# alexanderswerdlow/BEVGen

Measured on AMD Instinct MI355X. Metric: multi-view scenes/sec (6x256x256), higher is better.
Workload: dtype f32 (GEMM/conv/attention products as 3 f16 MFMAs on hi/lo splits, fp32 accumulate); 1 GPU; BASELINE configs[1]: Route M MaskGit, 6x256x256, batch 16 scenes/GPU, 18 iterations, + VQGAN decode to uint8; global_batch=16, parallelism=scene-parallel x1 (RCCL gather of uint8 pixels), precision_mode=f16x3

## Files before the change

### bevgen_amd/csrc/gemm_split_glds.hip

```cpp
#include "common.h"
#include "kernels.h"
#include "profiler.h"
#include <type_traits>
#include <vector>
#include <cstdio>

namespace bevgen {

typedef _Float16 half8 __attribute__((ext_vector_type(8)));
typedef unsigned u32x4 __attribute__((ext_vector_type(4)));

struct RowDiv {
    float d, r;
    __device__ __forceinline__ explicit RowDiv(float d_) : d(d_) {
        float r0 = __builtin_amdgcn_rcpf(d_);
        const float e = fmaf(-d_, r0, 1.0f);
        r0 = fmaf(e, r0, r0);
        const float e2 = fmaf(-d_, r0, 1.0f);
        r = fmaf(e2, r0, r0);
    }
    __device__ __forceinline__ float operator()(float x) const {
        const float q0 = x * r;
        const float e = fmaf(-d, q0, x);
        return fmaf(e, r, q0);
    }
};
constexpr int GBN = 128, GBK = 32;
#ifdef BEVGEN_GEMM_TRACE
__device__ unsigned long long g_gemm_trace[5 * 2048 * 8];
__device__ unsigned long long g_gemm_tr_tmp[2];
#define GT_STAMP(i) do { if (MODE == MODE_PLAIN && !KS) gt[i] = __builtin_amdgcn_s_memrealtime(); } while (0)
#else
#define GT_STAMP(i) do { } while (0)
#endif
constexpr float kGLoInv = 1.f / 2048.f;

__device__ __forceinline__ void glds16(const _Float16* src, _Float16* lds_wave_base) {
    __builtin_amdgcn_global_load_lds((const __attribute__((address_space(1))) void*)src, (__attribute__((address_space(3))) void*)lds_wave_base, 16, 0, 0);
}
__device__ __forceinline__ void glds16_buf(__amdgpu_buffer_rsrc_t rsrc, unsigned voff, int soff, _Float16* lds_wave_base) {
    __builtin_amdgcn_raw_ptr_buffer_load_lds(rsrc, (__attribute__((address_space(3))) void*)lds_wave_base, 16, (int)voff, soff, 0, 0);
}
template <int N>
__device__ __forceinline__ void wait_vmcnt() { asm volatile("s_waitcnt vmcnt(%0)" ::"n"(N) : "memory"); }
template <int DMA, int MAXN>
__device__ __forceinline__ void wait_tiles(int n) {
    if constexpr (MAXN <= 0) wait_vmcnt<0>();
    else {
        if (n >= MAXN) wait_vmcnt<MAXN * DMA>();
        else wait_tiles<DMA, MAXN - 1>(n);
    }
}

template <int DMA, int MAXN, int X>
__device__ __forceinline__ void wait_tiles_x(int n) {
    if constexpr (MAXN <= 0) wait_vmcnt<X>();
    else {
        if (n >= MAXN) wait_vmcnt<MAXN * DMA + X>();
        else wait_tiles_x<DMA, MAXN - 1, X>(n);
    }
}

template <int MODE, int WM, int S, bool W16, bool KS, int TI, int TJ, bool SKK = false>
__device__ __forceinline__ void gemm_tile(const GemmArgs& g, const int tx, const int ty, const int kt_first, const int nk, const int ksl, const int kz, const int sk_role,
                                          const int sk_first, const int tid
#ifdef BEVGEN_GEMM_TRACE
                                          , unsigned long long* gt
#endif
                                          ) {
    constexpr int TBM = WM * 64;
    constexpr int NW = WM * 8 / (TI * TJ);
    constexpr int WROWS = TI * 32;
    constexpr int WCOLS = TJ * 32;
    constexpr int WN = GBN / WCOLS;
    constexpr int NAJ = TBM / 8 / NW;
    constexpr int NBJ = 16 / NW;
    constexpr int AREGION = TBM * 2 * GBK;
    constexpr int STAGE_H = AREGION + GBN * 2 * GBK;
    constexpr int DMA = NAJ + NBJ;
    extern __shared__ __attribute__((aligned(1024))) _Float16 smem_g[];
    const int lane = tid & 63;
    const int wave = __builtin_amdgcn_readfirstlane(tid >> 6);
    const int wm = wave / WN, wn = wave % WN;
    const int r = lane & 31, h = lane >> 5;
    const int n0 = tx * GBN, m0 = ty * TBM + g.m_base;
    const int n0l = n0, m0l = m0;

    const _Float16* Ap = reinterpret_cast<const _Float16*>(g.A_hi);
    const _Float16* Bp = reinterpret_cast<const _Float16*>(g.B_hi);

    constexpr bool CONVG = MODE == MODE_CONV3, CONVS = MODE == MODE_CONV3S, CONV = CONVG || CONVS;
    unsigned a_off[NAJ], b_off[NBJ];
    int a_img[CONVG ? NAJ : 1], a_yx[CONVG ? NAJ : 1];
    unsigned a_msk[CONVS ? NAJ : 1];
#pragma unroll
    for (int j = 0; j < NBJ; ++j) {
        const int R = wave * (8 * NBJ) + j * 8 + (lane >> 3);
        const int c = (lane & 7) ^ ((R >> 1) & 7);
        const int n = min(n0l + R, g.N - 1);
        b_off[j] = (unsigned)(((long)n * 2 * g.ldb + c * 8) * 2);
    }
#pragma unroll
    for (int j = 0; j < NAJ; ++j) {
        const int R = wave * (8 * NAJ) + j * 8 + (lane >> 3);
        const int c = (lane & 7) ^ ((R >> 1) & 7);
        const int m = m0l + R;
        if constexpr (MODE == MODE_PLAIN) {
            a_off[j] = (unsigned)(((long)min(m, g.M - 1) * 2 * g.lda + c * 8) * 2);
        } else if constexpr (CONVS) {
            const int hw = g.conv_h * g.conv_w;
            const int mc = min(m, g.M - 1);
            const int img = mc / hw, rem = mc - img * hw;
            const int y = rem / g.conv_w, x = rem - y * g.conv_w;
            a_off[j] = (unsigned)mc * (unsigned)(g.conv_cin * 4) + (unsigned)(c * 16);
            unsigned rowm = (y > 0 ? 1u : 0u) | 2u | (y + 1 < g.conv_h ? 4u : 0u);
            unsigned colm = (x > 0 ? 1u : 0u) | 2u | (x + 1 < g.conv_w ? 4u : 0u);
            unsigned msk = 0;
#pragma unroll
            for (int kh = 0; kh < 3; ++kh)
                if (rowm & (1u << kh)) msk |= colm << (3 * kh);
            a_msk[j] = m < g.M ? msk : 0u;
        } else {
            a_off[j] = (unsigned)(c * 16);
            const int hw = g.conv_h * g.conv_w;
            const int img = m / hw, rem = m - img * hw;
            const int y = rem / g.conv_w;
            a_img[j] = img; a_yx[j] = (y << 16) | (rem - y * g.conv_w);
        }
    }
    int k_issue = kt_first * GBK;
    const int n_img = CONVG ? g.M / (g.conv_h * g.conv_w) : 0;
    const __amdgpu_buffer_rsrc_t a_rsrc = __builtin_amdgcn_make_buffer_rsrc(const_cast<_Float16*>(Ap), 0, CONV ? g.a_bytes : -1, 0x00020000);
    const __amdgpu_buffer_rsrc_t b_rsrc = __builtin_amdgcn_make_buffer_rsrc(const_cast<_Float16*>(Bp), 0, -1, 0x00020000);
    int s_c0 = 0, s_tap = 0;
    if (CONVS && kt_first > 0) { s_tap = k_issue / g.conv_cin; s_c0 = k_issue - s_tap * g.conv_cin; }
    auto tap_delta = [&]() { const int kh = s_tap / 3, kw = s_tap - 3 * kh; return ((kh - 1) * g.conv_w + (kw - 1)) * (g.conv_cin * 4) + s_c0 * 4; };
    int s_delta = CONVS ? tap_delta() : 0;
    unsigned s_bit = 1u << s_tap;
    auto issue_a = [&](int stage, int j) {
        _Float16* sa = smem_g + stage * STAGE_H + (wave * (8 * NAJ) + j * 8) * 2 * GBK;
        if constexpr (CONVS) {
            glds16_buf(a_rsrc, (a_msk[j] & s_bit) ? a_off[j] + (unsigned)s_delta : 0xFFFFFF00u, 0, sa);
        } else if constexpr (CONVG) {
            const int tap = k_issue / g.conv_cin;
            const int c0 = k_issue - tap * g.conv_cin;
            const int kh = tap / 3, kw = tap - kh * 3;
            int yy = (a_yx[j] >> 16) * g.conv_stride + kh - g.conv_pad, xx = (a_yx[j] & 0xffff) * g.conv_stride + kw - g.conv_pad;
            const int lim_h = g.conv_up ? 2 * g.conv_hin : g.conv_hin, lim_w = g.conv_up ? 2 * g.conv_win : g.conv_win;
            const bool ok = a_img[j] < n_img && yy >= 0 && yy < lim_h && xx >= 0 && xx < lim_w;
            if (g.conv_up) { yy >>= 1; xx >>= 1; }
            const unsigned off = (unsigned)((a_img[j] * g.conv_hin + yy) * g.conv_win + xx) * (unsigned)(g.conv_cin * 4) + (unsigned)(c0 * 4) + a_off[j];
            glds16_buf(a_rsrc, ok ? off : 0xFFFFFF00u, 0, sa);
        } else {
            glds16_buf(a_rsrc, a_off[j], k_issue * 4, sa);
        }
    };
    auto issue_b = [&](int stage) {
        _Float16* sb = smem_g + stage * STAGE_H + AREGION + wave * (8 * NBJ) * 2 * GBK;
#pragma unroll
        for (int j = 0; j < NBJ; ++j) glds16_buf(b_rsrc, b_off[j], k_issue * 4, sb + j * 8 * 2 * GBK);
        k_issue += GBK;
        if (CONVS) {
            s_c0 += GBK;
            s_delta += GBK * 4;
            if (s_c0 == g.conv_cin) { s_c0 = 0; ++s_tap; s_bit <<= 1; s_delta = tap_delta(); }
        }
    };
    auto issue_a_half = [&](int stage, int half) {
#pragma unroll
        for (int j = half * NAJ / 2; j < (half + 1) * NAJ / 2; ++j) issue_a(stage, j);
    };

    f32x16 accM[TI][TJ], accC[TI][TJ];
#pragma unroll
    for (int i = 0; i < TI; ++i)
#pragma unroll
        for (int j = 0; j < TJ; ++j)
#pragma unroll
            for (int q = 0; q < 16; ++q) { accM[i][j][q] = 0.f; accC[i][j][q] = 0.f; }

    int a_rd[2][2], b_rd[2][2];
#pragma unroll
    for (int i = 0; i < 2; ++i)
#pragma unroll
        for (int ks = 0; ks < 2; ++ks) {
            const int ra = wm * WROWS + (i < TI ? i : 0) * 32 + r, rb = wn * WCOLS + (i < TJ ? i : 0) * 32 + r;
            a_rd[i][ks] = ra * 2 * GBK + (((ks * 2 + h) ^ ((ra >> 1) & 7)) << 3);
            b_rd[i][ks] = AREGION + rb * 2 * GBK + (((ks * 2 + h) ^ ((rb >> 1) & 7)) << 3);
        }
    struct Frag { half8 ah[2], al[2], bh[2], bl[2]; };
    auto fetch = [&](Frag& f, int stage, int ks) {
        const _Float16* st = smem_g + stage * STAGE_H;
#pragma unroll
        for (int i = 0; i < 2; ++i) {
            if (i < TI) {
                f.ah[i] = *reinterpret_cast<const half8*>(st + a_rd[i][ks]);
                f.al[i] = *reinterpret_cast<const half8*>(st + (a_rd[i][ks] ^ 32));
            }
            if (i < TJ) {
                f.bh[i] = *reinterpret_cast<const half8*>(st + b_rd[i][ks]);
                if (!W16) f.bl[i] = *reinterpret_cast<const half8*>(st + (b_rd[i][ks] ^ 32));
            }
        }
    };
    auto mma_main = [&](const Frag& f) {
#pragma unroll
        for (int i = 0; i < TI; ++i)
#pragma unroll
            for (int j = 0; j < TJ; ++j) accM[i][j] = __builtin_amdgcn_mfma_f32_32x32x16_f16(f.bh[j], f.ah[i], accM[i][j], 0, 0, 0);
    };
    auto mma_c1 = [&](const Frag& f) {
        if (W16) return;
#pragma unroll
        for (int i = 0; i < TI; ++i)
#pragma unroll
            for (int j = 0; j < TJ; ++j) accC[i][j] = __builtin_amdgcn_mfma_f32_32x32x16_f16(f.bl[j], f.ah[i], accC[i][j], 0, 0, 0);
    };
    auto mma_c2 = [&](const Frag& f) {
#pragma unroll
        for (int i = 0; i < TI; ++i)
#pragma unroll
            for (int j = 0; j < TJ; ++j) accC[i][j] = __builtin_amdgcn_mfma_f32_32x32x16_f16(f.bh[j], f.al[i], accC[i][j], 0, 0, 0);
    };

#pragma unroll
    for (int s = 0; s < S; ++s)
        if (s < nk) { issue_a_half(s, 0); issue_a_half(s, 1); issue_b(s); }
    float* ln_rowstat = reinterpret_cast<float*>(smem_g + S * STAGE_H);
    if (MODE == MODE_PLAIN && g.ln_in_stats) {
        if (tid < TBM) {
            const int m = min(m0 + tid, g.M - 1);
            *reinterpret_cast<float2*>(ln_rowstat + tid * 2) = reinterpret_cast<const float2*>(g.ln_in_stats)[m];
        }
    } else if (MODE == MODE_PLAIN && g.ln_in_gsums) {
        constexpr int NT = NW * 64, PARTS = NT / TBM;
        static_assert(NT % TBM == 0, "threads per block row");
        const int row = tid % TBM, part = tid / TBM;
        const int m = min(m0 + row, g.M - 1);
        const float2* st = reinterpret_cast<const float2*>(g.ln_in_gsums) + m;
        const int G = g.ln_in_groups;
        double s1 = 0.0, s2 = 0.0;
        for (int g0 = part; g0 < G; g0 += 16 * PARTS) {
            float2 v[16];
#pragma unroll
            for (int u = 0; u < 16; ++u) v[u] = st[(long)min(g0 + u * PARTS, G - 1) * g.ln_rows];
#pragma unroll
            for (int u = 0; u < 16; ++u)
                if (g0 + u * PARTS < G) { s1 += (double)v[u].x; s2 += (double)v[u].y; }
        }
        double* partial = reinterpret_cast<double*>(reinterpret_cast<char*>(smem_g + S * STAGE_H) + 6144);
        partial[(part * TBM + row) * 2] = s1;
        partial[(part * TBM + row) * 2 + 1] = s2;
        __syncthreads();
        if (tid < TBM) {
            double t1 = 0.0, t2 = 0.0;
#pragma unroll
            for (int pp = 0; pp < PARTS; ++pp) { t1 += partial[(pp * TBM + tid) * 2]; t2 += partial[(pp * TBM + tid) * 2 + 1]; }
            const double mean = t1 / (double)g.ln_in_count;
            const double var = fmax(t2 / (double)g.ln_in_count - mean * mean, 0.0);
            *reinterpret_cast<float2*>(ln_rowstat + tid * 2) = make_float2((float)mean, (float)(1.0 / sqrt(var + (double)g.ln_eps)));
        }
    }
    wait_tiles<DMA, S - 1>(nk - 1);
    __builtin_amdgcn_s_barrier();
    asm volatile("" ::: "memory");
    GT_STAMP(1);
    Frag f0, f1;
    fetch(f0, 0, 0);

    constexpr bool RPF = MODE == MODE_PLAIN && TI == 2 && TJ == 2 && !KS && !SKK;
    constexpr int RPF_N = 2;
    const bool rpf_on = RPF && g.r_prefetch && sk_role == 0 && nk >= S;
    bool rpf_pending = false, rpf_flight = false;
    auto issue_rpf = [&](int stg) {
        const __amdgpu_buffer_rsrc_t r_rsrc = __builtin_amdgcn_make_buffer_rsrc(const_cast<float*>(g.R), 0, -1, 0x00020000);
        const int row = min(m0 + wm * WROWS + lane, g.M - 1);
        const int col = min(n0 + wn * WCOLS, g.N - 64);
        const unsigned off = (unsigned)(((long)row * g.ldr + col) * 4);
        _Float16* dst = smem_g + S * STAGE_H + 2048;
        (void)stg;
        glds16_buf(r_rsrc, off, 0, dst);
        glds16_buf(r_rsrc, off + 128u, 0, dst + 512);
    };
    int stage = 0;
    auto body = [&](auto where_c, auto steady_c, int kt) {
        constexpr int WHERE = decltype(where_c)::value;
        constexpr bool STEADY = decltype(steady_c)::value;
        const int stage_next = stage == S - 1 ? 0 : stage + 1;
        const int stage_prev = stage == 0 ? S - 1 : stage - 1;
#define BG_FENCE() __builtin_amdgcn_sched_barrier(0)
        fetch(f1, stage, 1);
        BG_FENCE();
        mma_main(f0);
        BG_FENCE();
        if (WHERE == 2) { issue_a_half(stage_prev, 0); BG_FENCE(); }
        mma_c1(f0);
        BG_FENCE();
        if (WHERE == 2) { issue_a_half(stage_prev, 1); BG_FENCE(); }
        mma_c2(f0);
        if (WHERE == 2) { BG_FENCE(); issue_b(stage_prev); }
        __builtin_amdgcn_sched_barrier(0);
        asm volatile("s_waitcnt lgkmcnt(0)" ::: "memory");
        if (STEADY) wait_vmcnt<(S - 2) * DMA>();
        else if (RPF && rpf_flight) wait_tiles_x<DMA, S - 2, RPF_N>(nk - kt - 2);
        else wait_tiles<DMA, S - 2>(nk - kt - 2);
        __builtin_amdgcn_s_barrier();
        asm volatile("" ::: "memory");
        __builtin_amdgcn_sched_barrier(0);
        mma_main(f1);
        __builtin_amdgcn_sched_barrier(0);
        fetch(f0, stage_next, 0);
        BG_FENCE();
        if (WHERE == 1) { issue_a_half(stage, 0); BG_FENCE(); }
        if (RPF && WHERE == 0 && rpf_pending) { issue_rpf(stage); rpf_pending = false; rpf_flight = true; BG_FENCE(); }
        mma_c1(f1);
        BG_FENCE();
        if (WHERE == 1) { issue_a_half(stage, 1); BG_FENCE(); }
        mma_c2(f1);
        BG_FENCE();
        if (WHERE == 1) { issue_b(stage); BG_FENCE(); }
#undef BG_FENCE
        stage = stage_next;
    };
    using std::integral_constant;
    const bool late = NW == 8 && wave >= NW / 2;
    int kt = 0;
    if (!late) {
        for (; kt < nk - S; ++kt) body(integral_constant<int, 1>{}, integral_constant<bool, true>{}, kt);
    } else {
        if (nk > 0) { body(integral_constant<int, 0>{}, integral_constant<bool, false>{}, 0); kt = 1; }
        for (; kt <= nk - S; ++kt) body(integral_constant<int, 2>{}, integral_constant<bool, true>{}, kt);
    }
    rpf_pending = rpf_on;
    for (; kt < nk; ++kt) body(integral_constant<int, 0>{}, integral_constant<bool, false>{}, kt);
    GT_STAMP(2);

    if (MODE == MODE_PLAIN && sk_role != 0) {
        constexpr int SLOT = NW * TI * TJ * 16 * 64;
        float* ws = reinterpret_cast<float*>(g.sk_ws) + 1024;
        unsigned* flags = reinterpret_cast<unsigned*>(g.sk_ws);
        const long lane_off = (long)wave * (TI * TJ * 16 * 64) + lane * 4;
        if (sk_role == 1) {
            float* mine = ws + (long)blockIdx.x * SLOT + lane_off;
#pragma unroll
            for (int i = 0; i < TI; ++i)
#pragma unroll
                for (int j = 0; j < TJ; ++j)
#pragma unroll
                    for (int qq = 0; qq < 4; ++qq) {
                        f32x4 v;
#pragma unroll
                        for (int e = 0; e < 4; ++e) v[e] = accM[i][j][qq * 4 + e] + accC[i][j][qq * 4 + e] * kGLoInv;
                        *reinterpret_cast<f32x4*>(mine + ((i * TJ + j) * 4 + qq) * 256) = v;
                    }
            asm volatile("s_waitcnt vmcnt(0)" ::: "memory");
            __syncthreads();
            if (tid == 0) __hip_atomic_store(flags + blockIdx.x, g.sk_epoch, __ATOMIC_RELAXED, __HIP_MEMORY_SCOPE_AGENT);
            return;
        }
        if (tid == 0) {
            const long long t_in = __builtin_amdgcn_s_memrealtime();
            for (int w = sk_first; w < (int)blockIdx.x; w += 8)
                while (__hip_atomic_load(flags + w, __ATOMIC_RELAXED, __HIP_MEMORY_SCOPE_AGENT) != g.sk_epoch) {
                    __builtin_amdgcn_s_sleep(1);
                    if (__builtin_amdgcn_s_memrealtime() - t_in > 200LL * 1000 * 100) { status_raise(g.status, BG_ST_MLP_BARRIER); break; }
                }
        }
        __syncthreads();
#pragma unroll
        for (int i = 0; i < TI; ++i)
#pragma unroll
            for (int j = 0; j < TJ; ++j)
#pragma unroll
                for (int q = 0; q < 16; ++q) { accM[i][j][q] += accC[i][j][q] * kGLoInv; accC[i][j][q] = 0.f; }
        for (int w = (int)blockIdx.x - 8; w >= sk_first; w -= 8) {
            const float* theirs = ws + (long)w * SLOT + lane_off;
            constexpr int NQ = TI * TJ * 4, HB = NQ >= 8 ? 8 : NQ;
#pragma unroll
            for (int u0 = 0; u0 < NQ; u0 += HB) {
                f32x4 pv[HB];
#pragma unroll
                for (int u = 0; u < HB; ++u) asm volatile("global_load_dwordx4 %0, %1, off sc1" : "=v"(pv[u]) : "v"(theirs + (u0 + u) * 256) : "memory");
                asm volatile("s_waitcnt vmcnt(0)" ::: "memory");
#pragma unroll
                for (int u = 0; u < HB; ++u) {
                    asm volatile("" : "+v"(pv[u]));
                    const int uu = u0 + u;
#pragma unroll
                    for (int e = 0; e < 4; ++e) accM[uu / (TJ * 4)][(uu / 4) % TJ][(uu & 3) * 4 + e] += pv[u][e];
                }
            }
        }
    }
    if (MODE == MODE_PLAIN && (g.ln_in_stats || g.ln_in_gsums)) {
        float ln_mean[TI], ln_rstd[TI];
#pragma unroll
        for (int i = 0; i < TI; ++i) { const float2 mr = *reinterpret_cast<const float2*>(ln_rowstat + (wm * WROWS + i * 32 + r) * 2); ln_mean[i] = mr.x; ln_rstd[i] = mr.y; }
#pragma unroll
        for (int i = 0; i < TI; ++i)
#pragma unroll
            for (int j = 0; j < TJ; ++j)
#pragma unroll
                for (int qq = 0; qq < 4; ++qq) {
                    const int n = min(n0 + wn * WCOLS + j * 32 + 8 * qq + 4 * h, g.N - 4);
                    const f32x4 cs = *reinterpret_cast<const f32x4*>(g.ln_in_cs + n);
#pragma unroll
                    for (int e = 0; e < 4; ++e) {
                        const int q = qq * 4 + e;
                        accM[i][j][q] = ln_rstd[i] * ((accM[i][j][q] + accC[i][j][q] * kGLoInv) - ln_mean[i] * cs[e]);
                        accC[i][j][q] = 0.f;
                    }
                }
    }
    constexpr int VT_LD = WROWS == 64 ? 72 : 40;
    constexpr int RS = TJ == 2 ? 68 : 36;
    constexpr int SLICE_W = TJ == 2 ? (64 * VT_LD > WROWS * RS ? 64 * VT_LD : WROWS * RS) : WROWS * RS;
    constexpr bool STG = MODE == MODE_PLAIN && !KS && !SKK && !(WM == 2 && S == 2) && (TI == 2 ? TJ == 2 : true) && (long)NW * SLICE_W * 4 <= (long)S * STAGE_H * 2;
    float* const pl = reinterpret_cast<float*>(smem_g) + wave * SLICE_W;
    const int rm_row = lane >> 3, rm_c8 = lane & 7;
    auto stage_read8 = [&](int row, f32x4& a0, f32x4& a1) {
        a0 = *reinterpret_cast<const f32x4*>(pl + row * RS + 8 * rm_c8);
        a1 = *reinterpret_cast<const f32x4*>(pl + row * RS + 8 * rm_c8 + 4);
    };
    auto split8 = [&](const f32x4& a0, const f32x4& a1, half8& hi8, half8& lo8) {
#pragma unroll
        for (int e = 0; e < 4; ++e) {
            hi8[e] = split_hi(a0[e]); lo8[e] = split_lo(a0[e], hi8[e]);
            hi8[4 + e] = split_hi(a1[e]); lo8[4 + e] = split_lo(a1[e], hi8[4 + e]);
        }
    };
    if constexpr (TJ == 2) {
    if (MODE == MODE_PLAIN && g.epi != EPI_PLAIN && n0 + wn * 64 >= g.N) return;
    const bool qkv = MODE == MODE_PLAIN && g.epi == EPI_MUSE_QKV;
    if (g.epi == EPI_MUSE_Q || (qkv && n0 + wn * 64 < g.epi_heads * 64)) {
        _Float16* Qh = reinterpret_cast<_Float16*>(qkv ? g.epi_qh : g.epi_hi);
        _Float16* Ql = reinterpret_cast<_Float16*>(qkv ? g.epi_ql : g.epi_lo);
        const float* qsc = qkv ? g.epi_qscale : g.epi_scale;
        const int head = (n0 + wn * 64) >> 6;
        unsigned bad = 0;
        f32x4 qsc4[2][4];
#pragma unroll
        for (int j = 0; j < 2; ++j)
#pragma unroll
            for (int qq = 0; qq < 4; ++qq) qsc4[j][qq] = *reinterpret_cast<const f32x4*>(qsc + j * 32 + 8 * qq + 4 * h);
        if constexpr (STG) {
            if (g.row_major_epi) {
#pragma unroll
                for (int i = 0; i < TI; ++i) {
                    float v[2][16];
                    float ss = 0.f;
#pragma unroll
                    for (int j = 0; j < 2; ++j)
#pragma unroll
                        for (int q = 0; q < 16; ++q) {
                            v[j][q] = (accM[i][j][q] + accC[i][j][q] * kGLoInv) * g.alpha * 8.0f;
                            ss = fmaf(v[j][q], v[j][q], ss);
                        }
                    ss += xor32(ss);
                    const float nrm = fmaxf(sqrtf(ss), 1e-12f);
                    const RowDiv rdiv(nrm);
#pragma unroll
                    for (int j = 0; j < 2; ++j)
#pragma unroll
                        for (int qq = 0; qq < 4; ++qq) {
                            const f32x4 sc = qsc4[j][qq];
                            f32x4 o;
#pragma unroll
                            for (int e = 0; e < 4; ++e) o[e] = (rdiv(v[j][qq * 4 + e]) * sc[e]) * g.epi_post;
                            *reinterpret_cast<f32x4*>(pl + (i * 32 + r) * RS + j * 32 + 8 * qq + 4 * h) = o;
                        }
                }
#pragma unroll
                for (int ps = 0; ps < WROWS / 8; ++ps) {
                    const int row = ps * 8 + rm_row, m = m0 + wm * WROWS + row;
                    f32x4 a0, a1;
                    stage_read8(row, a0, a1);
                    half8 hi8, lo8;
                    split8(a0, a1, hi8, lo8);
                    if (m < g.M) {
                        guard_half8(hi8, bad);
                        const int bb = m / g.epi_rows, nq = m - bb * g.epi_rows;
                        const long dst = (((long)bb * g.epi_heads + head) * g.epi_rows + nq) * 64 + 8 * rm_c8;
                        *reinterpret_cast<half8*>(Qh + dst) = hi8;
                        *reinterpret_cast<half8*>(Ql + dst) = lo8;
                    }
                }
                if (bad) status_raise(g.status, BG_ST_F16_RANGE);
                return;
            }
        }
#pragma unroll
        for (int i = 0; i < TI; ++i) {
            const int m = m0 + wm * WROWS + i * 32 + r;
            float v[2][16];
            float ss = 0.f;
#pragma unroll
            for (int j = 0; j < 2; ++j)
#pragma unroll
                for (int q = 0; q < 16; ++q) {
                    v[j][q] = (accM[i][j][q] + accC[i][j][q] * kGLoInv) * g.alpha * 8.0f;
                    ss = fmaf(v[j][q], v[j][q], ss);
                }
            ss += xor32(ss);
            const float nrm = fmaxf(sqrtf(ss), 1e-12f);
                    const RowDiv rdiv(nrm);
            if (m >= g.M) continue;
            const int bb = m / g.epi_rows, nq = m - bb * g.epi_rows;
            const long dst = (((long)bb * g.epi_heads + head) * g.epi_rows + nq) * 64;
#pragma unroll
            for (int j = 0; j < 2; ++j)
#pragma unroll
                for (int qq = 0; qq < 4; ++qq) {
                    const int d = j * 32 + 8 * qq + 4 * h;
                    const f32x4 sc = qsc4[j][qq];
                    half4_t hi4, lo4;
#pragma unroll
                    for (int e = 0; e < 4; ++e) {
                        const float qv = (rdiv(v[j][qq * 4 + e]) * sc[e]) * g.epi_post;
                        hi4[e] = split_hi(qv);
                        lo4[e] = split_lo(qv, hi4[e]);
                    }
                    guard_half4(hi4, bad);
                    *reinterpret_cast<half4_t*>(Qh + dst + d) = hi4;
                    *reinterpret_cast<half4_t*>(Ql + dst + d) = lo4;
                }
        }
        if (bad) status_raise(g.status, BG_ST_F16_RANGE);
        return;
    }
    if (MODE == MODE_PLAIN && (g.epi == EPI_MUSE_KV || qkv)) {
        const int HD = g.epi_heads * 64;
        const int ncol = n0 + wn * 64 - (qkv ? HD : 0);
        const bool is_v = ncol >= HD;
        const int head = (is_v ? ncol - HD : ncol) >> 6;
        const _Float16* aux = reinterpret_cast<const _Float16*>(g.epi_aux);
        unsigned bad = 0;
        f32x4 ksc4[2][4];
#pragma unroll
        for (int j = 0; j < 2; ++j)
#pragma unroll
            for (int qq = 0; qq < 4; ++qq) ksc4[j][qq] = *reinterpret_cast<const f32x4*>(g.epi_scale + j * 32 + 8 * qq + 4 * h);
        if constexpr (STG) {
            const int prow0 = m0 + wm * WROWS;
            if (g.row_major_epi && is_v && (g.epi_rows % WROWS) == 0 && (g.epi_ld & 7) == 0 && prow0 + WROWS <= g.M) {
                unsigned* plu = reinterpret_cast<unsigned*>(pl);
#pragma unroll
                for (int i = 0; i < TI; ++i)
#pragma unroll
                    for (int j = 0; j < 2; ++j)
#pragma unroll
                        for (int q = 0; q < 16; ++q) {
                            const float val = (accM[i][j][q] + accC[i][j][q] * kGLoInv) * g.alpha;
                            const _Float16 hi = split_hi(val);
                            const _Float16 lo = split_lo(val, hi);
                            const int d = j * 32 + (q & 3) + 8 * (q >> 2) + 4 * h;
                            plu[d * VT_LD + 1 + i * 32 + r] = (unsigned)__builtin_bit_cast(unsigned short, hi) | ((unsigned)__builtin_bit_cast(unsigned short, lo) << 16);
                        }
                const int bb = prow0 / g.epi_rows, nk0 = prow0 - bb * g.epi_rows;
                _Float16* Vh = reinterpret_cast<_Float16*>(g.epi_hi2);
                _Float16* Vl = reinterpret_cast<_Float16*>(g.epi_lo2);
                constexpr int G8 = WROWS / 8;
                const int gq = lane % G8;
#pragma unroll
                for (int ps = 0; ps < G8; ++ps) {
                    const int d = ps * (64 / G8) + lane / G8;
                    const u32x4 u0 = *reinterpret_cast<const u32x4*>(plu + d * VT_LD + 8 * gq);
                    const u32x4 u1 = *reinterpret_cast<const u32x4*>(plu + d * VT_LD + 8 * gq + 4);
                    u32x4 hw, lw;
                    hw[0] = __builtin_amdgcn_perm(u0[1], u0[0], 0x05040100u); lw[0] = __builtin_amdgcn_perm(u0[1], u0[0], 0x07060302u);
                    hw[1] = __builtin_amdgcn_perm(u0[3], u0[2], 0x05040100u); lw[1] = __builtin_amdgcn_perm(u0[3], u0[2], 0x07060302u);
                    hw[2] = __builtin_amdgcn_perm(u1[1], u1[0], 0x05040100u); lw[2] = __builtin_amdgcn_perm(u1[1], u1[0], 0x07060302u);
                    hw[3] = __builtin_amdgcn_perm(u1[3], u1[2], 0x05040100u); lw[3] = __builtin_amdgcn_perm(u1[3], u1[2], 0x07060302u);
                    const long rowp = (((long)bb * g.epi_heads + head) * 64 + d) * g.epi_ld + nk0 + 8 * gq;
                    if (gq == 0) {
                        if (nk0 == 0) {
                            hw[0] = (hw[0] & 0xFFFF0000u) | (unsigned)__builtin_bit_cast(unsigned short, aux[2 * HD + head * 64 + d]);
                            lw[0] = (lw[0] & 0xFFFF0000u) | (unsigned)__builtin_bit_cast(unsigned short, aux[3 * HD + head * 64 + d]);
                            bad |= f16x2_nonfinite(hw[0] & 0xFFFF0000u) | f16x2_nonfinite(hw[1]) | f16x2_nonfinite(hw[2]) | f16x2_nonfinite(hw[3]);
                            *reinterpret_cast<u32x4*>(Vh + rowp) = hw;
                            *reinterpret_cast<u32x4*>(Vl + rowp) = lw;
                        } else {
                            bad |= f16x2_nonfinite(hw[0] & 0xFFFF0000u) | f16x2_nonfinite(hw[1]) | f16x2_nonfinite(hw[2]) | f16x2_nonfinite(hw[3]);
                            *reinterpret_cast<unsigned short*>(Vh + rowp + 1) = (unsigned short)(hw[0] >> 16);
                            *reinterpret_cast<unsigned short*>(Vl + rowp + 1) = (unsigned short)(lw[0] >> 16);
                            *reinterpret_cast<unsigned*>(Vh + rowp + 2) = hw[1];
                            *reinterpret_cast<unsigned*>(Vl + rowp + 2) = lw[1];
                            *reinterpret_cast<uint2*>(Vh + rowp + 4) = make_uint2(hw[2], hw[3]);
                            *reinterpret_cast<uint2*>(Vl + rowp + 4) = make_uint2(lw[2], lw[3]);
                        }
                    } else {
                        bad |= f16x2_nonfinite(hw[0]) | f16x2_nonfinite(hw[1]) | f16x2_nonfinite(hw[2]) | f16x2_nonfinite(hw[3]);
                        *reinterpret_cast<u32x4*>(Vh + rowp) = hw;
                        *reinterpret_cast<u32x4*>(Vl + rowp) = lw;
                        if (gq == 1) {
                            const unsigned ut = plu[d * VT_LD + WROWS];
                            bad |= f16x2_nonfinite(ut & 0xFFFFu);
                            const long tp = (((long)bb * g.epi_heads + head) * 64 + d) * g.epi_ld + nk0 + WROWS;
                            *reinterpret_cast<unsigned short*>(Vh + tp) = (unsigned short)(ut & 0xFFFFu);
                            *reinterpret_cast<unsigned short*>(Vl + tp) = (unsigned short)(ut >> 16);
                        }
                    }
                }
                if (bad) status_raise(g.status, BG_ST_F16_RANGE);
                return;
            }
            if (g.row_major_epi && !is_v) {
                _Float16* Kh = reinterpret_cast<_Float16*>(g.epi_hi);
                _Float16* Kl = reinterpret_cast<_Float16*>(g.epi_lo);
#pragma unroll
                for (int i = 0; i < TI; ++i) {
                    float v[2][16];
                    float ss = 0.f;
#pragma unroll
                    for (int j = 0; j < 2; ++j)
#pragma unroll
                        for (int q = 0; q < 16; ++q) {
                            v[j][q] = (accM[i][j][q] + accC[i][j][q] * kGLoInv) * g.alpha;
                            ss = fmaf(v[j][q], v[j][q], ss);
                        }
                    ss += xor32(ss);
                    const float nrm = fmaxf(sqrtf(ss), 1e-12f);
                    const RowDiv rdiv(nrm);
#pragma unroll
                    for (int j = 0; j < 2; ++j)
#pragma unroll
                        for (int qq = 0; qq < 4; ++qq) {
                            const f32x4 sc = ksc4[j][qq];
                            f32x4 o;
#pragma unroll
                            for (int e = 0; e < 4; ++e) o[e] = rdiv(v[j][qq * 4 + e]) * sc[e];
                            *reinterpret_cast<f32x4*>(pl + (i * 32 + r) * RS + j * 32 + 8 * qq + 4 * h) = o;
                        }
                }
#pragma unroll
                for (int ps = 0; ps < WROWS / 8; ++ps) {
                    const int row = ps * 8 + rm_row, m = m0 + wm * WROWS + row;
                    f32x4 a0, a1;
                    stage_read8(row, a0, a1);
                    half8 hi8, lo8;
                    split8(a0, a1, hi8, lo8);
                    if (m < g.M) {
                        guard_half8(hi8, bad);
                        const int bb = m / g.epi_rows, nk = m - bb * g.epi_rows;
                        const long dst = (((long)bb * g.epi_heads + head) * g.epi_ld + 1 + nk) * 64 + 8 * rm_c8;
                        *reinterpret_cast<half8*>(Kh + dst) = hi8;
                        *reinterpret_cast<half8*>(Kl + dst) = lo8;
                        if (nk == 0) {
                            *reinterpret_cast<half8*>(Kh + dst - 64) = *reinterpret_cast<const half8*>(aux + head * 64 + 8 * rm_c8);
                            *reinterpret_cast<half8*>(Kl + dst - 64) = *reinterpret_cast<const half8*>(aux + HD + head * 64 + 8 * rm_c8);
                        }
                    }
                }
                if (bad) status_raise(g.status, BG_ST_F16_RANGE);
                return;
            }
        }
#pragma unroll
        for (int i = 0; i < TI; ++i) {
            const int m = m0 + wm * WROWS + i * 32 + r;
            const int mc = min(m, g.M - 1);
            const int bb = mc / g.epi_rows, nk = mc - bb * g.epi_rows;
            float v[2][16];
            float ss = 0.f;
#pragma unroll
            for (int j = 0; j < 2; ++j)
#pragma unroll
                for (int q = 0; q < 16; ++q) {
                    v[j][q] = (accM[i][j][q] + accC[i][j][q] * kGLoInv) * g.alpha;
                    ss = fmaf(v[j][q], v[j][q], ss);
                }
            ss += xor32(ss);
            if (m >= g.M) continue;
            if (!is_v) {
                const float nrm = fmaxf(sqrtf(ss), 1e-12f);
                    const RowDiv rdiv(nrm);
                _Float16* Kh = reinterpret_cast<_Float16*>(g.epi_hi);
                _Float16* Kl = reinterpret_cast<_Float16*>(g.epi_lo);
                const long dst = (((long)bb * g.epi_heads + head) * g.epi_ld + 1 + nk) * 64;
#pragma unroll
                for (int j = 0; j < 2; ++j)
#pragma unroll
                    for (int qq = 0; qq < 4; ++qq) {
                        const int d = j * 32 + 8 * qq + 4 * h;
                        const f32x4 sc = ksc4[j][qq];
                        half4_t hi4, lo4;
#pragma unroll
                        for (int e = 0; e < 4; ++e) {
                            const float kv = rdiv(v[j][qq * 4 + e]) * sc[e];
                            hi4[e] = split_hi(kv);
                            lo4[e] = split_lo(kv, hi4[e]);
                        }
                        guard_half4(hi4, bad);
                        *reinterpret_cast<half4_t*>(Kh + dst + d) = hi4;
                        *reinterpret_cast<half4_t*>(Kl + dst + d) = lo4;
                        if (nk == 0) {
                            *reinterpret_cast<half4_t*>(Kh + dst - (long)64 + d) = *reinterpret_cast<const half4_t*>(aux + head * 64 + d);
                            *reinterpret_cast<half4_t*>(Kl + dst - (long)64 + d) = *reinterpret_cast<const half4_t*>(aux + HD + head * 64 + d);
                        }
                    }
            } else {
                _Float16* Vh = reinterpret_cast<_Float16*>(g.epi_hi2);
                _Float16* Vl = reinterpret_cast<_Float16*>(g.epi_lo2);
                const long base = ((long)bb * g.epi_heads + head) * 64 * g.epi_ld + 1 + nk;
#pragma unroll
                for (int j = 0; j < 2; ++j)
#pragma unroll
                    for (int q = 0; q < 16; ++q) {
                        const int d = j * 32 + (q & 3) + 8 * (q >> 2) + 4 * h;
                        const _Float16 hi = split_hi(v[j][q]);
                        guard_half(hi, bad);
                        Vh[base + (long)d * g.epi_ld] = hi;
                        Vl[base + (long)d * g.epi_ld] = split_lo(v[j][q], hi);
                        if (nk == 0) {
                            Vh[base - 1 + (long)d * g.epi_ld] = aux[2 * HD + head * 64 + d];
                            Vl[base - 1 + (long)d * g.epi_ld] = aux[3 * HD + head * 64 + d];
                        }
                    }
            }
        }
        if (bad) status_raise(g.status, BG_ST_F16_RANGE);
        return;
// ... 395 lines not shown
```

Measured before the change: 11.25 scenes/s.

## Switch split-f16 GEMM main loop from 32x32x16 to 16x16x32 MFMA tiles

Replaces the 32x32x16 MFMA inner loop with 16x16x32 MFMAs on 16-row fragments, restructuring fragment fetches, the interleaving with DMA issue, and the stream-K partial store and reduce. Before the existing epilogues run, the 16x16 accumulators are shuffled through LDS back into the 32x32 accumulator layout, so those epilogues stay unchanged. The aim is better MFMA throughput and finer interleaving of LDS reads with MFMAs. The cost is an extra LDS round trip and barrier in the epilogue, plus more accumulator registers during the conversion.

New measurement: 11.52 scenes/s, median of 6. 2.4% higher.

```diff
diff --git a/bevgen_amd/csrc/gemm_split_glds.hip b/bevgen_amd/csrc/gemm_split_glds.hip
--- a/bevgen_amd/csrc/gemm_split_glds.hip
+++ b/bevgen_amd/csrc/gemm_split_glds.hip
@@ -26,6 +26,9 @@
     }
 };
 constexpr int GBN = 128, GBK = 32;
+#ifndef BEVGEN_GEMM_MFMA16
+#define BEVGEN_GEMM_MFMA16 1
+#endif
 #ifdef BEVGEN_GEMM_TRACE
 __device__ unsigned long long g_gemm_trace[5 * 2048 * 8];
 __device__ unsigned long long g_gemm_tr_tmp[2];
@@ -79,10 +82,10 @@
     constexpr int STAGE_H = AREGION + GBN * 2 * GBK;
     constexpr int DMA = NAJ + NBJ;
     extern __shared__ __attribute__((aligned(1024))) _Float16 smem_g[];
-    const int lane = tid & 63;
+    int lane = tid & 63;
     const int wave = __builtin_amdgcn_readfirstlane(tid >> 6);
     const int wm = wave / WN, wn = wave % WN;
-    const int r = lane & 31, h = lane >> 5;
+    int r = lane & 31, h = lane >> 5;
     const int n0 = tx * GBN, m0 = ty * TBM + g.m_base;
     const int n0l = n0, m0l = m0;
 
@@ -179,6 +182,50 @@
 #pragma unroll
             for (int q = 0; q < 16; ++q) { accM[i][j][q] = 0.f; accC[i][j][q] = 0.f; }
 
+#if BEVGEN_GEMM_MFMA16
+    constexpr int NI = 2 * TI, NJ = 2 * TJ;
+    constexpr int T16 = 16 * 2 * GBK;
+    f32x4 qM[NI][NJ], qC[NI][NJ];
+#pragma unroll
+    for (int i = 0; i < NI; ++i)
+#pragma unroll
+        for (int j = 0; j < NJ; ++j)
+#pragma unroll
+            for (int e = 0; e < 4; ++e) { qM[i][j][e] = 0.f; qC[i][j][e] = 0.f; }
+    const int r16 = lane & 15, c16 = lane >> 4;
+    const int a_rd = (wm * WROWS + r16) * 2 * GBK + ((c16 ^ (((wm * WROWS + r16) >> 1) & 7)) << 3);
+    const int b_rd = AREGION + (wn * WCOLS + r16) * 2 * GBK + ((c16 ^ (((wn * WCOLS + r16) >> 1) & 7)) << 3);
+    struct AFrag { half8 h[TI], l[TI]; };
+    half8 bh[NJ], bl[NJ];
+    auto fetch_a = [&](AFrag& f, int stage, int half) {
+        const int hi = stage * STAGE_H + a_rd, lo = hi ^ 32;
+#pragma unroll
+        for (int i = 0; i < TI; ++i) {
+            f.h[i] = *reinterpret_cast<const half8*>(smem_g + hi + (half * TI + i) * T16);
+            f.l[i] = *reinterpret_cast<const half8*>(smem_g + lo + (half * TI + i) * T16);
+        }
+    };
+    auto fetch_b = [&](int stage, int jg) {
+        const int hi = stage * STAGE_H + b_rd, lo = hi ^ 32;
+#pragma unroll
+        for (int j = 0; j < TJ; ++j) {
+            bh[jg * TJ + j] = *reinterpret_cast<const half8*>(smem_g + hi + (jg * TJ + j) * T16);
+            if (!W16) bl[jg * TJ + j] = *reinterpret_cast<const half8*>(smem_g + lo + (jg * TJ + j) * T16);
+        }
+    };
+    auto mma = [&](const AFrag& a, int half, int jg, int part) {
+        if (part == 1 && W16) return;
+#pragma unroll
+        for (int jj = 0; jj < TJ; ++jj)
+#pragma unroll
+            for (int i = 0; i < TI; ++i) {
+                const int it = half * TI + i, j = jg * TJ + jj;
+                if (part == 0) qM[it][j] = __builtin_amdgcn_mfma_f32_16x16x32_f16(bh[j], a.h[i], qM[it][j], 0, 0, 0);
+                else if (part == 1) qC[it][j] = __builtin_amdgcn_mfma_f32_16x16x32_f16(bl[j], a.h[i], qC[it][j], 0, 0, 0);
+                else qC[it][j] = __builtin_amdgcn_mfma_f32_16x16x32_f16(bh[j], a.l[i], qC[it][j], 0, 0, 0);
+            }
+    };
+#else
     int a_rd[2][2], b_rd[2][2];
 #pragma unroll
     for (int i = 0; i < 2; ++i)
@@ -222,6 +269,7 @@
 #pragma unroll
             for (int j = 0; j < TJ; ++j) accC[i][j] = __builtin_amdgcn_mfma_f32_32x32x16_f16(f.bh[j], f.al[i], accC[i][j], 0, 0, 0);
     };
+#endif
 
 #pragma unroll
     for (int s = 0; s < S; ++s)
@@ -265,8 +313,13 @@
     __builtin_amdgcn_s_barrier();
     asm volatile("" ::: "memory");
     GT_STAMP(1);
+#if BEVGEN_GEMM_MFMA16
+    AFrag fa0, fa1;
+    auto first_fetch = [&]() { fetch_b(0, 0); fetch_b(0, 1); fetch_a(fa0, 0, 0); };
+#else
     Frag f0, f1;
     fetch(f0, 0, 0);
+#endif
 
     constexpr bool RPF = MODE == MODE_PLAIN && TI == 2 && TJ == 2 && !KS && !SKK;
     constexpr int RPF_N = 2;
@@ -289,6 +342,21 @@
         const int stage_next = stage == S - 1 ? 0 : stage + 1;
         const int stage_prev = stage == 0 ? S - 1 : stage - 1;
 #define BG_FENCE() __builtin_amdgcn_sched_barrier(0)
+#if BEVGEN_GEMM_MFMA16
+        fetch_a(fa1, stage, 1);
+        BG_FENCE();
+        mma(fa0, 0, 0, 0);
+        mma(fa0, 0, 0, 1);
+        BG_FENCE();
+        if (WHERE == 2) { issue_a_half(stage_prev, 0); BG_FENCE(); }
+        mma(fa0, 0, 0, 2);
+        mma(fa0, 0, 1, 0);
+        BG_FENCE();
+        if (WHERE == 2) { issue_a_half(stage_prev, 1); BG_FENCE(); }
+        mma(fa0, 0, 1, 1);
+        mma(fa0, 0, 1, 2);
+        if (WHERE == 2) { BG_FENCE(); issue_b(stage_prev); }
+#else
         fetch(f1, stage, 1);
         BG_FENCE();
         mma_main(f0);
@@ -299,6 +367,7 @@
         if (WHERE == 2) { issue_a_half(stage_prev, 1); BG_FENCE(); }
         mma_c2(f0);
         if (WHERE == 2) { BG_FENCE(); issue_b(stage_prev); }
+#endif
         __builtin_amdgcn_sched_barrier(0);
         asm volatile("s_waitcnt lgkmcnt(0)" ::: "memory");
         if (STEADY) wait_vmcnt<(S - 2) * DMA>();
@@ -307,6 +376,27 @@
         __builtin_amdgcn_s_barrier();
         asm volatile("" ::: "memory");
         __builtin_amdgcn_sched_barrier(0);
+#if BEVGEN_GEMM_MFMA16
+        mma(fa1, 1, 0, 0);
+        __builtin_amdgcn_sched_barrier(0);
+        fetch_a(fa0, stage_next, 0);
+        BG_FENCE();
+        if (WHERE == 1) { issue_a_half(stage, 0); BG_FENCE(); }
+        if (RPF && WHERE == 0 && rpf_pending) { issue_rpf(stage); rpf_pending = false; rpf_flight = true; BG_FENCE(); }
+        mma(fa1, 1, 0, 1);
+        mma(fa1, 1, 0, 2);
+        BG_FENCE();
+        fetch_b(stage_next, 0);
+        BG_FENCE();
+        if (WHERE == 1) { issue_a_half(stage, 1); BG_FENCE(); }
+        mma(fa1, 1, 1, 0);
+        mma(fa1, 1, 1, 1);
+        mma(fa1, 1, 1, 2);
+        BG_FENCE();
+        fetch_b(stage_next, 1);
+        BG_FENCE();
+        if (WHERE == 1) { issue_b(stage); BG_FENCE(); }
+#else
         mma_main(f1);
         __builtin_amdgcn_sched_barrier(0);
         fetch(f0, stage_next, 0);
@@ -319,6 +409,7 @@
         mma_c2(f1);
         BG_FENCE();
         if (WHERE == 1) { issue_b(stage); BG_FENCE(); }
+#endif
 #undef BG_FENCE
         stage = stage_next;
     };
@@ -326,8 +417,16 @@
     const bool late = NW == 8 && wave >= NW / 2;
     int kt = 0;
     if (!late) {
+#if BEVGEN_GEMM_MFMA16
+        asm volatile("; early waves" ::: "memory");
+        first_fetch();
+#endif
         for (; kt < nk - S; ++kt) body(integral_constant<int, 1>{}, integral_constant<bool, true>{}, kt);
     } else {
+#if BEVGEN_GEMM_MFMA16
+        asm volatile("; late waves" ::: "memory");
+        first_fetch();
+#endif
         if (nk > 0) { body(integral_constant<int, 0>{}, integral_constant<bool, false>{}, 0); kt = 1; }
         for (; kt <= nk - S; ++kt) body(integral_constant<int, 2>{}, integral_constant<bool, true>{}, kt);
     }
@@ -342,6 +441,15 @@
         const long lane_off = (long)wave * (TI * TJ * 16 * 64) + lane * 4;
         if (sk_role == 1) {
             float* mine = ws + (long)blockIdx.x * SLOT + lane_off;
+#if BEVGEN_GEMM_MFMA16
+#pragma unroll
+            for (int u = 0; u < NI * NJ; ++u) {
+                f32x4 v;
+#pragma unroll
+                for (int e = 0; e < 4; ++e) v[e] = qM[u / NJ][u % NJ][e] + qC[u / NJ][u % NJ][e] * kGLoInv;
+                *reinterpret_cast<f32x4*>(mine + u * 256) = v;
+            }
+#else
 #pragma unroll
             for (int i = 0; i < TI; ++i)
 #pragma unroll
@@ -353,6 +461,7 @@
                         for (int e = 0; e < 4; ++e) v[e] = accM[i][j][qq * 4 + e] + accC[i][j][qq * 4 + e] * kGLoInv;
                         *reinterpret_cast<f32x4*>(mine + ((i * TJ + j) * 4 + qq) * 256) = v;
                     }
+#endif
             asm volatile("s_waitcnt vmcnt(0)" ::: "memory");
             __syncthreads();
             if (tid == 0) __hip_atomic_store(flags + blockIdx.x, g.sk_epoch, __ATOMIC_RELAXED, __HIP_MEMORY_SCOPE_AGENT);
@@ -367,12 +476,19 @@
                 }
         }
         __syncthreads();
+#if BEVGEN_GEMM_MFMA16
+#pragma unroll
+        for (int u = 0; u < NI * NJ; ++u)
+#pragma unroll
+            for (int e = 0; e < 4; ++e) { qM[u / NJ][u % NJ][e] += qC[u / NJ][u % NJ][e] * kGLoInv; qC[u / NJ][u % NJ][e] = 0.f; }
+#else
 #pragma unroll
         for (int i = 0; i < TI; ++i)
 #pragma unroll
             for (int j = 0; j < TJ; ++j)
 #pragma unroll
                 for (int q = 0; q < 16; ++q) { accM[i][j][q] += accC[i][j][q] * kGLoInv; accC[i][j][q] = 0.f; }
+#endif
         for (int w = (int)blockIdx.x - 8; w >= sk_first; w -= 8) {
             const float* theirs = ws + (long)w * SLOT + lane_off;
             constexpr int NQ = TI * TJ * 4, HB = NQ >= 8 ? 8 : NQ;
@@ -387,11 +503,54 @@
                     asm volatile("" : "+v"(pv[u]));
                     const int uu = u0 + u;
 #pragma unroll
+#if BEVGEN_GEMM_MFMA16
+                    for (int e = 0; e < 4; ++e) qM[uu / NJ][uu % NJ][e] += pv[u][e];
+#else
                     for (int e = 0; e < 4; ++e) accM[uu / (TJ * 4)][(uu / 4) % TJ][(uu & 3) * 4 + e] += pv[u][e];
-                }
-            }
-        }
-    }
+#endif
+                }
+            }
+        }
+    }
+    constexpr int VT_LD = WROWS == 64 ? 72 : 40;
+    constexpr int RS = TJ == 2 ? 68 : 36;
+    constexpr int SLICE_W = TJ == 2 ? (64 * VT_LD > WROWS * RS ? 64 * VT_LD : WROWS * RS) : WROWS * RS;
+    constexpr bool STG = MODE == MODE_PLAIN && !KS && !SKK && !(WM == 2 && S == 2) && (TI == 2 ? TJ == 2 : true) && (long)NW * SLICE_W * 4 <= (long)S * STAGE_H * 2;
+    float* const pl = reinterpret_cast<float*>(smem_g) + wave * SLICE_W;
+#if BEVGEN_GEMM_MFMA16
+    lane = (int)__builtin_amdgcn_mbcnt_hi(~0u, __builtin_amdgcn_mbcnt_lo(~0u, 0u));
+    r = lane & 31; h = lane >> 5;
+    {
+        constexpr bool CV_FULL = (long)NW * SLICE_W * 4 <= (long)S * STAGE_H * 2;
+        constexpr int CV_W = CV_FULL ? SLICE_W : 32 * RS;
+        static_assert((long)NW * CV_W * 4 <= (long)S * STAGE_H * 2, "the ring holds a 32-row half of every wave's patch");
+        static_assert(!STG || CV_FULL, "the staged epilogues' slice is the conversion's slice");
+        if constexpr (!STG) __syncthreads();
+        const int wr = (lane & 15) * RS + 4 * (lane >> 4), rd = r * RS + 4 * h;
+        float* const cv = reinterpret_cast<float*>(smem_g) + wave * CV_W;
+#pragma unroll
+        for (int i = 0; i < TI; ++i) {
+            float* const ch = cv + (CV_FULL ? i * 32 * RS : 0);
+#pragma unroll
+            for (int t = 0; t < 2; ++t)
+#pragma unroll
+                for (int j = 0; j < NJ; ++j) {
+                    f32x4 v;
+#pragma unroll
+                    for (int e = 0; e < 4; ++e) v[e] = fmaf(qC[2 * i + t][j][e], kGLoInv, qM[2 * i + t][j][e]);
+                    *reinterpret_cast<f32x4*>(ch + wr + t * 16 * RS + j * 16) = v;
+                }
+#pragma unroll
+            for (int j = 0; j < TJ; ++j)
+#pragma unroll
+                for (int qq = 0; qq < 4; ++qq) {
+                    const f32x4 v = *reinterpret_cast<const f32x4*>(ch + rd + j * 32 + 8 * qq);
+#pragma unroll
+                    for (int e = 0; e < 4; ++e) { accM[i][j][qq * 4 + e] = v[e]; accC[i][j][qq * 4 + e] = 0.f; }
+                }
+        }
+    }
+#endif
     if (MODE == MODE_PLAIN && (g.ln_in_stats || g.ln_in_gsums)) {
         float ln_mean[TI], ln_rstd[TI];
 #pragma unroll
@@ -412,11 +571,6 @@
                     }
                 }
     }
-    constexpr int VT_LD = WROWS == 64 ? 72 : 40;
-    constexpr int RS = TJ == 2 ? 68 : 36;
-    constexpr int SLICE_W = TJ == 2 ? (64 * VT_LD > WROWS * RS ? 64 * VT_LD : WROWS * RS) : WROWS * RS;
-    constexpr bool STG = MODE == MODE_PLAIN && !KS && !SKK && !(WM == 2 && S == 2) && (TI == 2 ? TJ == 2 : true) && (long)NW * SLICE_W * 4 <= (long)S * STAGE_H * 2;
-    float* const pl = reinterpret_cast<float*>(smem_g) + wave * SLICE_W;
     const int rm_row = lane >> 3, rm_c8 = lane & 7;
     auto stage_read8 = [&](int row, f32x4& a0, f32x4& a1) {
         a0 = *reinterpret_cast<const f32x4*>(pl + row * RS + 8 * rm_c8);
```
